# y-scope/pinot

Hardware: AMD Instinct MI355X
Metric: scanned rows/sec + achieved HBM GB/s, filtered SUM on 1B-row segment (higher is better)
Workload: dtype int64

## Files before the change

pinot_amd/csrc/pg_device.h:

```cpp
#pragma once
#include <stdint.h>

namespace pg {

constexpr int kWave = 64;
constexpr int kMaxTileSteps = 32;
constexpr int kMaxTileDocs = kWave * kMaxTileSteps;
constexpr int kMaxCols = 16;
constexpr int kMaxLeaves = 8;
constexpr int kMaxNodes = 24;
constexpr int kMaxAggCols = 4;
constexpr int kMaxGroupCols = 10;
constexpr int kMaxHashLevels = 8;
constexpr int kMaxGroupAggs = 8;
constexpr int kStackDepth = 8;
constexpr int kSetLdsWords = 2048;
constexpr int kBlockThreads = 256;
constexpr int kWideBlockThreads = 640;
constexpr int kHistBlockThreads = 1024;
constexpr unsigned long long kPartialHistAlarm = 1ull;
constexpr unsigned long long kPartialStale = 2ull;
constexpr int kGroupBlockThreads = 1024;

enum LeafKind : int32_t {
// ... 124 lines not shown
struct ScanParams {
  int32_t num_docs;
  int32_t num_tiles;
  int32_t tile_steps;
  int32_t num_cols;
  int32_t num_leaves;
  int32_t num_nodes;
  int32_t num_agg_cols;
  int32_t num_bitmap_leaves;
  int32_t stage_bytes;
  int32_t queue_off;
  int32_t queue_cap;
  int32_t wave_lds_bytes;
  int32_t speculate;
  int32_t double_buffer;
  int32_t lazy_columns;
  int32_t lazy_node;
  int32_t profile;
  int32_t bitmap_off;
  int32_t bitmap_bytes;
  int32_t num_stage;
  int32_t hist_slot;
  int32_t hist_bins;
  DevStage stage[kMaxCols];
  DevNode nodes[kMaxNodes];
  DevAggCol agg_cols[kMaxAggCols];
  const unsigned long long* bitmaps[kMaxLeaves];
  int32_t bitmap_lds_off[kMaxLeaves];
  const uint32_t* tile_list;
  const uint32_t* tile_count;
  int32_t raw64_coalesced;
  int32_t lane_skip;
  unsigned long long* filter_entries;
  unsigned long long* out_bitmap;
  BlockPartial* partials;
  uint32_t* done_counter;
  struct HostRecord* host_out;
  unsigned long long host_seq;
  int32_t fold_slots;
  int32_t fold_typed;
  int32_t sparse_lanes;
  int32_t fold_one_counter;
  uint8_t* leap_tables;
  uint32_t* leaf_out[kMaxLeaves];
  int32_t leaf_out_enabled;
  uint32_t* fsm_tables;
  int32_t fsm_states, fsm_inputs;
  int8_t fsm_input_of_leaf[kMaxLeaves];
  const struct WindowInfo* sparse_windows;
  int32_t sparse_num_windows;
  int32_t set_leaves_in_lds;
  uint8_t fsm_delta[64];
  int32_t lean_kind;
};

constexpr int kMaxDistinctKeys = 4;
struct DistinctCol {
  const uint8_t* fwd;
  uint32_t* set_bits;
  int32_t bits;
  int32_t words;
  int32_t lds_off;
  int32_t pad;
};
struct DistinctKey {
  const uint8_t* fwd;
  int32_t bits;
  uint32_t mult;
};
struct DistinctParams {
  ScanParams scan;
  int32_t num_cols;
  int32_t num_keys;
  int32_t lds_words;
  int32_t pad;
  DistinctCol cols[kMaxAggCols];
  DistinctKey keys[kMaxDistinctKeys];
};

struct CollectParams {
  DistinctParams d;
  const uint8_t* fwd[kMaxAggCols];
  int32_t vkind[kMaxAggCols];
  unsigned long long* out_images[kMaxAggCols];
  uint32_t* out_rows;
  unsigned long long* cursor;
  uint32_t* flags;
  unsigned long long capacity;
};
constexpr uint32_t kCollectOverflow = 1u;

struct HllParams {
  DistinctParams d;
  const uint8_t* fwd[kMaxAggCols];
  uint32_t* regs[kMaxAggCols];
  int32_t wide[kMaxAggCols];
  int32_t log2m[kMaxAggCols];
  int32_t lds_off[kMaxAggCols];
  int32_t lds_words;
  uint32_t num_rows;
};
enum HllDictKind : int32_t { kHllDictI32 = 0, kHllDictI64 = 1, kHllDictFloat = 2, kHllDictDouble = 3 };
struct HllFoldParams {
  const uint32_t* bits;
  uint32_t* regs;
  const int32_t* dict32;
// ... 186 lines not shown
```

pinot_amd/csrc/pg_dma_pairs.h:

```cpp
#pragma once
#include <cstddef>

namespace pg {

constexpr int kDmaMaxBits = 20;
constexpr int kDmaSlotsPerWave = 2;
constexpr int kDmaWavesPerBlock = 4;
constexpr int kDmaRecordBytes = 1024;
constexpr size_t kDmaLdsBudget = 156 * 1024;
constexpr int kDmaMinSlotBytes = 6912;
constexpr int kDmaBlocksPerCu = 2;

constexpr int dma_pieces(int bits) { return (bits + 3) / 4; }
constexpr int dma_last_lanes(int bits) { return 16 * (bits - 4 * (dma_pieces(bits) - 1)); }
constexpr int dma_instructions(int filter_bits, int value_bits) { return dma_pieces(filter_bits) + dma_pieces(value_bits); }
constexpr int dma_slot_bytes(int filter_bits, int value_bits) { return 256 * (filter_bits + value_bits); }
constexpr size_t dma_lds_bytes(int filter_bits, int value_bits, int slots, int waves) {
  return (size_t)kDmaRecordBytes + (size_t)waves * slots * dma_slot_bytes(filter_bits, value_bits);
}

constexpr bool dma_width(int bits) { return bits >= 1 && bits <= kDmaMaxBits; }
constexpr bool dma_pair_admitted(int filter_bits, int value_bits) {
  return dma_width(filter_bits) && dma_width(value_bits) && dma_slot_bytes(filter_bits, value_bits) >= kDmaMinSlotBytes &&
         kDmaLdsBudget / dma_lds_bytes(filter_bits, value_bits, kDmaSlotsPerWave, kDmaWavesPerBlock) >= (size_t)kDmaBlocksPerCu;
}
constexpr int dma_pair_index(int filter_bits, int value_bits) {
  if (!dma_pair_admitted(filter_bits, value_bits)) return -1;
  int at = 0;
  for (int f = 1; f <= kDmaMaxBits; ++f)
    for (int v = 1; v <= kDmaMaxBits; ++v) {
      if (f == filter_bits && v == value_bits) return at;
      if (dma_pair_admitted(f, v)) ++at;
    }
  return -1;
}
constexpr int dma_pair_count() {
  int n = 0;
  for (int f = 1; f <= kDmaMaxBits; ++f)
    for (int v = 1; v <= kDmaMaxBits; ++v) n += dma_pair_admitted(f, v) ? 1 : 0;
  return n;
}
constexpr int kDmaPairs = dma_pair_count();
constexpr int dma_pair_at(int index) {
  int at = 0;
  for (int f = 1; f <= kDmaMaxBits; ++f)
    for (int v = 1; v <= kDmaMaxBits; ++v)
      if (dma_pair_admitted(f, v) && at++ == index) return f * 32 + v;
  return 0;
}
static_assert(kDmaPairs == 102, "27 <= f + v <= 38, both up to 20 bits");
static_assert(dma_pair_admitted(10, 17) && dma_pair_admitted(7, 20) && dma_pair_admitted(20, 18) && !dma_pair_admitted(6, 20) && !dma_pair_admitted(19, 20), "the rule's edges");

}
```

pinot_amd/csrc/pg_engine.hip:

```cpp
#include <hip/hip_runtime.h>

#include <algorithm>
#include <chrono>
#include <array>
#include <atomic>
#include <condition_variable>
#include <functional>
#include <memory>
#include <cmath>
#include <cstdarg>
#include <cstdio>
#include <cstdlib>
#include <cstring>
#include <limits>
#include <mutex>
#include <string>
#include <thread>
#include <vector>

#include "../../include/pinot_gpu.h"
#include "pg_device.h"
#include "pg_filter_stats.h"
#include "pg_filter_fsm.h"
#include "pg_fsm_kernels.h"
#include "pg_kernels.h"
#include "pg_launch.h"
#include "pg_rank_image.h"
#include "pg_raw_set_table.h"
#include "pg_hll.h"
#include "pg_set_pass_layout.h"
#include "pg_group_plan.h"
#include "pg_dma_pairs.h"
#include "pg_chunk_decode.h"

namespace {

using namespace pg;

thread_local std::string g_error;

pg_status fail(pg_status st, const char* fmt, ...) {
  char buf[1024];
  va_list ap;
  va_start(ap, fmt);
  vsnprintf(buf, sizeof(buf), fmt, ap);
  va_end(ap);
  g_error = buf;
  return st;
}

#define HIP_TRY(expr)                                                                                  \
  do {                                                                                                 \
    hipError_t _e = (expr);                                                                            \
    if (_e != hipSuccess)                                                                              \
      return fail(_e == hipErrorOutOfMemory ? PG_ERR_OUT_OF_MEMORY : PG_ERR_DEVICE, "%s failed: %s (%s:%d)", #expr, \
                  hipGetErrorString(_e), __FILE__, __LINE__);                                          \
  } while (0)

struct Engine {
  bool initialized = false;
  std::atomic<uint64_t> epoch{0};
  int device = 0;
  int blocks_per_cu = 0;
  bool raw64_coalesced = true;
  int wide_plane = -1;
  bool partition_stats_cache = true;
  bool partition_packed = true;
  bool plane_async = true;
  bool staged_h2d = true;
  long long exact_stats_docs = 64ll << 20;
  int flags = 0;
  bool use_dma = true;
  int value_plane = -1;
  int tile_steps = 0;
  bool double_buffer = false;
  bool direct_result = true;
  int fold_finalize = -1;
  int fold_one_counter = 1;
  bool poll_result = true;
  bool distinct_lds = true;
  bool collect = false;
  bool chunk_decode_host = false;
  bool percentile_lds = true;
  bool set_lds = true;
  bool lane_skip = true;
  bool batch_blocks_per_cu_forced = false;
  int batch_blocks_per_cu = 4;
  bool scan_raw = true;
  bool scan_raw_set = true;
  int scan_simple_valid = 1;
  int scan_simple_pipe = 1;
  int scan_simple_dma = 1;
  int dma_pair = 1;
  int dma_nt = -1;
  int dma_blocks_per_cu = 0;
  bool scan_simple = true;
  bool scan_sparse = true;
  bool lean_batch = true;
  bool partition_two_level = true;
  bool fsm_perm = true;
  int index_and_waves = 0;
  bool batch_index = true;
  bool index_gather = true;
  bool fsm_fused = true;
  bool fsm_stats = true;
  bool fsm_episodes = true;
  bool plan_cache = true;
  bool group_publish = true;
  bool batch_more = true;
  bool group_one_launch = true;
  bool batch_group = true;
  bool batch_hist = true;
  bool batch_launch = true;
  bool leap2 = true;
  int sparse_lanes = 32;
  bool plane_gcd = true;
  bool scan_private = true;
  bool group_private = true;
  int group_log_replicas = 3;
  bool group_pack = true;
  bool scan_typed_private = true;
  bool scan_narrow_single = true;
  bool scan_narrow = true;
  bool group_partition = true;
  long long partition_min_docs = 1ll << 22;
  unsigned long long group_table_bytes = 64ull << 30;
  int hist = -1;
  int hist_blocks = 0;
  bool hist_guard = false;
  int hist_bits = 0;
// ... 146 lines not shown
  mutable std::mutex doc_sets_mu;
  std::vector<std::shared_ptr<DocSet>> doc_sets;
};


struct FsmSide {
  const pg::fstats::Fsm* fsm = nullptr;
  uint32_t* bitmap[pg::kFsmInputs] = {};
  bool mapped[pg::kFsmInputs] = {};
  bool kernel_wrote = false;
  uint32_t* tables = nullptr;
  uint32_t* chunks = nullptr;
  unsigned long long* entries = nullptr;
  long long num_tiles = 0, num_chunks = 0;
  bool fused = false;
  bool prepared = false;
};
constexpr size_t kAndShardBytes = (size_t)pg::kAndCardinalityShards * 128;
constexpr size_t kFsmStageBytes = 64 + (1 + (size_t)fstats::kFsmMaxEpisodeStreams) * ((size_t)pg::kFsmStates << pg::kFsmInputs);

namespace {

void destroy_ctx(ExecCtx* c) {
  if (!c) return;
  if (c->stream) (void)hipStreamSynchronize(c->stream);
  if (c->h_fsm_stage) (void)hipHostFree(c->h_fsm_stage);
  if (c->d_fsm_scratch) (void)hipFree(c->d_fsm_scratch);
  for (hipEvent_t e : c->ev_pass) if (e) (void)hipEventDestroy(e);
  if (c->d_partials) (void)hipFree(c->d_partials);
  if (c->h_record) (void)hipHostFree(c->h_record);
  if (c->d_done) (void)hipFree(c->d_done);
  for (auto* b : c->d_bitmaps) (void)hipFree(b);
  for (auto* s : c->d_sets) (void)hipFree(s);
  if (c->d_table) (void)hipFree(c->d_table);
  if (c->h_table) (void)hipHostFree(c->h_table);
  if (c->d_gather_in) (void)hipFree(c->d_gather_in);
  if (c->d_gather_out) (void)hipFree(c->d_gather_out);
  if (c->d_partition) (void)hipFree(c->d_partition);
  if (c->d_tile_list) (void)hipFree(c->d_tile_list);
  if (c->d_and_counters) (void)hipFree(c->d_and_counters);
  if (c->h_and_shards) (void)hipHostFree(c->h_and_shards);
  if (c->d_window_info) (void)hipFree(c->d_window_info);
  if (c->d_distinct) (void)hipFree(c->d_distinct);
  if (c->d_arena) (void)hipFree(c->d_arena);
  if (c->h_groups) (void)hipHostFree(c->h_groups);
  if (c->d_filter_entries) (void)hipFree(c->d_filter_entries);
  if (c->d_leap_tables) (void)hipFree(c->d_leap_tables);
  if (c->h_filter_entries) (void)hipHostFree(c->h_filter_entries);
  for (auto& e : c->ev) if (e) (void)hipEventDestroy(e);
  if (c->stream) (void)hipStreamDestroy(c->stream);
  delete c;
}

pg_status acquire_ctx(pg_segment* seg, ExecCtx** out) {
  {
    std::lock_guard<std::mutex> lk(seg->ctx_mu);
    if (!seg->free_ctx.empty()) {
      *out = seg->free_ctx.back();
      seg->free_ctx.pop_back();
      return PG_OK;
    }
  }
  ExecCtx* c = new ExecCtx();
  hipError_t e = hipStreamCreateWithFlags(&c->stream, hipStreamNonBlocking);
  if (e == hipSuccess) for (auto& ev : c->ev) { e = hipEventCreate(&ev); if (e != hipSuccess) break; }
  if (e == hipSuccess) e = hipHostMalloc((void**)&c->h_record, sizeof(HostRecord), hipHostMallocMapped);
  if (e == hipSuccess) { memset(c->h_record, 0, sizeof(HostRecord)); c->h_partial = &c->h_record->partial; }
  if (e == hipSuccess) e = hipHostGetDevicePointer((void**)&c->h_record_dev, c->h_record, 0);
  if (e == hipSuccess) e = hipMalloc((void**)&c->d_done, 10 * 128);
  if (e == hipSuccess) e = hipMemsetAsync(c->d_done, 0, 10 * 128, c->stream);
  if (e != hipSuccess) {
    destroy_ctx(c);
    return fail(PG_ERR_DEVICE, "creating execution context failed: %s", hipGetErrorString(e));
  }
  {
    std::lock_guard<std::mutex> lk(seg->ctx_mu);
    seg->all_ctx.push_back(c);
  }
  *out = c;
  return PG_OK;
}

void release_ctx(pg_segment* seg, ExecCtx* c) {
  std::lock_guard<std::mutex> lk(seg->ctx_mu);
  seg->free_ctx.push_back(c);
}

struct CtxGuard {
  pg_segment* seg;
  ExecCtx* ctx;
  ~CtxGuard() { if (ctx) release_ctx(seg, ctx); }
};

pg_status ensure_partials(ExecCtx* c, int blocks) {
  if (c->partial_capacity >= blocks + kFoldExtraRecords) return PG_OK;
  if (c->d_partials) (void)hipFree(c->d_partials);
  c->d_partials = nullptr;
  HIP_TRY(hipMalloc((void**)&c->d_partials, sizeof(BlockPartial) * (size_t)(blocks + kFoldExtraRecords)));
  c->partial_capacity = blocks + kFoldExtraRecords;
  return PG_OK;
}

pg_status ensure_bitmap(pg_segment* seg, ExecCtx* c, size_t index) {
  while (c->d_bitmaps.size() <= index) {
    unsigned long long* p = nullptr;
    size_t words = (size_t)std::max(seg->num_tiles, 1) * kMaxTileSteps;
    HIP_TRY(hipMalloc((void**)&p, words * 8));
    c->d_bitmaps.push_back(p);
  }
  return PG_OK;
}

constexpr size_t kDistinctKeepWords = (size_t)64 << 20;
pg_status ensure_distinct(pg_segment* seg, ExecCtx* c, size_t words) {
  if (c->distinct_capacity >= words) return PG_OK;
  if (c->d_distinct) { (void)hipFree(c->d_distinct); seg->device_bytes -= c->distinct_capacity * 4; }
  c->d_distinct = nullptr; c->distinct_capacity = 0;
  HIP_TRY(hipMalloc((void**)&c->d_distinct, words * 4));
  c->distinct_capacity = words;
  seg->device_bytes += words * 4;
  return PG_OK;
}
void trim_distinct(pg_segment* seg, ExecCtx* c) {
// ... 1338 lines not shown
#else
  std::this_thread::yield();
#endif
}

template <typename Done>
pg_status wait_polled(hipStream_t stream, long long docs, Done&& done) {
  long long spins = 0;
  std::chrono::steady_clock::time_point until;
  while (!done()) {
    cpu_relax();
    if ((++spins & 0x3FF) != 0) continue;
    const auto now = std::chrono::steady_clock::now();
    if (spins == 0x400) { until = now + std::chrono::nanoseconds(300'000 + docs / 1000); continue; }
    if (now >= until || hipStreamQuery(stream) != hipErrorNotReady) { HIP_TRY(hipStreamSynchronize(stream)); break; }
  }
  __atomic_thread_fence(__ATOMIC_ACQUIRE);
  return PG_OK;
}

}

extern "C" {

const char* pg_last_error(void) { return g_error.c_str(); }
const char* pg_version(void) { return "pinot_amd 0.1 (gfx950)"; }

pg_status pg_init(const pg_config* config) {
  std::lock_guard<std::mutex> lk(g_engine.mu);
  if (config && config->abi_version != PG_ABI_VERSION) return fail(PG_ERR_INVALID_ARGUMENT, "ABI version mismatch: got %d, built %d", config->abi_version, PG_ABI_VERSION);
  int count = 0;
  hipError_t e = hipGetDeviceCount(&count);
  if (e != hipSuccess || count == 0) return fail(PG_ERR_DEVICE, "no HIP device available: %s", hipGetErrorString(e));
  g_engine.physical_devices = count;
  const char* ald = getenv("PINOT_GPU_ALIAS_DEVICES");
  g_engine.logical_devices = (ald && atoi(ald) > count) ? std::min(atoi(ald), 64) : count;
  int dev = config ? config->device_id : 0;
  if (dev < 0 || dev >= g_engine.logical_devices) return fail(PG_ERR_INVALID_ARGUMENT, "device %d out of range (have %d)", dev, g_engine.logical_devices);
  g_engine.device = dev;
  g_engine.blocks_per_cu = config ? config->blocks_per_cu : 0;
  g_engine.flags = config ? config->flags : 0;
  const char* nodma = getenv("PINOT_GPU_NO_DMA");
  g_engine.use_dma = !(nodma && nodma[0] == '1');
  const char* vp = getenv("PINOT_GPU_VALUE_PLANE");
  g_engine.value_plane = vp ? atoi(vp) : -1;
  const char* db = getenv("PINOT_GPU_DOUBLE_BUFFER");
  g_engine.double_buffer = db && db[0] == '1';
  const char* drv = getenv("PINOT_GPU_DIRECT_RESULT");
  g_engine.direct_result = !(drv && drv[0] == '0');
  const char* ffz = getenv("PINOT_GPU_FOLD_FINALIZE");
  g_engine.fold_finalize = ffz ? (ffz[0] == '0' ? 0 : 1) : -1;
  const char* foc = getenv("PINOT_GPU_FOLD_ONE_COUNTER");
  g_engine.fold_one_counter = foc ? (foc[0] == '0' ? 0 : 1) : 1;
  const char* prs = getenv("PINOT_GPU_POLL_RESULT");
  g_engine.poll_result = !(prs && prs[0] == '0');
  const char* lsk = getenv("PINOT_GPU_LANE_SKIP");
  g_engine.lane_skip = !(lsk && lsk[0] == '0');
  const char* bbc = getenv("PINOT_GPU_BATCH_BLOCKS_PER_CU");
  g_engine.batch_blocks_per_cu_forced = bbc != nullptr;
  g_engine.batch_blocks_per_cu = (bbc && atoi(bbc) > 0) ? atoi(bbc) : 4;
  const char* ssp = getenv("PINOT_GPU_SCAN_SPARSE");
  g_engine.scan_sparse = !(ssp && ssp[0] == '0');
  const char* ssm = getenv("PINOT_GPU_SCAN_SIMPLE");
  g_engine.scan_simple = !(ssm && ssm[0] == '0');
  const char* ssv = getenv("PINOT_GPU_SCAN_SIMPLE_VALID");
  g_engine.scan_simple_valid = ssv ? (ssv[0] == '0' ? 0 : (ssv[0] == '2' ? 2 : 1)) : 1;
  const char* spp = getenv("PINOT_GPU_SCAN_SIMPLE_PIPE");
  g_engine.scan_simple_pipe = spp ? (spp[0] == '0' ? 0 : (spp[0] == '2' ? 2 : 1)) : 1;
  const char* sdm = getenv("PINOT_GPU_SCAN_SIMPLE_DMA");
  g_engine.scan_simple_dma = sdm ? (sdm[0] == '0' ? 0 : (sdm[0] == '2' ? 2 : 1)) : 1;
  const char* sdp = getenv("PINOT_GPU_SCAN_SIMPLE_DMA_PAIR");
  g_engine.dma_pair = sdp && sdp[0] == '0' ? 0 : 1;
  const char* sdn = getenv("PINOT_GPU_SCAN_SIMPLE_DMA_NT");
  g_engine.dma_nt = sdn ? (sdn[0] == '0' ? 0 : 1) : -1;
  const char* sdb = getenv("PINOT_GPU_SCAN_SIMPLE_DMA_BLOCKS_PER_CU");
  g_engine.dma_blocks_per_cu = sdb && atoi(sdb) > 0 ? atoi(sdb) : 0;
  const char* srw = getenv("PINOT_GPU_SCAN_RAW");
  g_engine.scan_raw = !(srw && srw[0] == '0');
  const char* srs = getenv("PINOT_GPU_SCAN_RAW_SET");
  g_engine.scan_raw_set = !(srs && srs[0] == '0');
  const char* bla = getenv("PINOT_GPU_BATCH_LAUNCH");
  g_engine.batch_launch = !(bla && bla[0] == '0');
  auto env_on = [](const char* name) { const char* v = getenv(name); return !(v && v[0] == '0'); };
  g_engine.lean_batch = env_on("PINOT_GPU_LEAN_BATCH");
  g_engine.set_lds = env_on("PINOT_GPU_SET_LDS");
  g_engine.distinct_lds = env_on("PINOT_GPU_DISTINCT_LDS");
  g_engine.percentile_lds = env_on("PINOT_GPU_PERCENTILE_LDS");
  { const char* cv = getenv("PINOT_GPU_COLLECT"); g_engine.collect = cv != nullptr && cv[0] == '1'; }
  { const char* cd = getenv("PINOT_GPU_CHUNK_DECODE"); g_engine.chunk_decode_host = cd != nullptr && strcmp(cd, "host") == 0; }
  g_engine.partition_two_level = env_on("PINOT_GPU_PARTITION_TWO_LEVEL");
  g_engine.fsm_perm = env_on("PINOT_GPU_FSM_PERM");
  g_engine.fsm_stats = env_on("PINOT_GPU_FSM_STATS");
  g_engine.fsm_fused = env_on("PINOT_GPU_FSM_FUSED");
  g_engine.fsm_episodes = env_on("PINOT_GPU_FSM_EPISODES");
  g_engine.index_gather = env_on("PINOT_GPU_INDEX_GATHER");
  g_engine.batch_index = env_on("PINOT_GPU_BATCH_INDEX");
  { const char* iaw = getenv("PINOT_GPU_INDEX_AND_WAVES"); g_engine.index_and_waves = iaw ? std::max(-64, std::min(32, atoi(iaw))) : 0; }
  g_engine.group_one_launch = env_on("PINOT_GPU_GROUP_ONE_LAUNCH");
  g_engine.plan_cache = env_on("PINOT_GPU_PLAN_CACHE");
  g_engine.group_publish = env_on("PINOT_GPU_GROUP_PUBLISH");
  const char* bmo = getenv("PINOT_GPU_BATCH_MORE");
  g_engine.batch_more = !(bmo && bmo[0] == '0');
  const char* bgr = getenv("PINOT_GPU_BATCH_GROUP");
  g_engine.batch_group = !(bgr && bgr[0] == '0');
  const char* bhi = getenv("PINOT_GPU_BATCH_HIST");
  g_engine.batch_hist = !(bhi && bhi[0] == '0');
// ... 1768 lines not shown
      const int ac = agg_slot_of[(size_t)a];
      const ColumnDev& col = seg->cols[(size_t)ag.column];
      const bool plane = lw.plane_cols[(size_t)ag.column] != 0;
      const bool raw = col.encoding == PG_FWD_RAW_FIXED_BYTE;
      if (ag.function == PG_AGG_SUM || ag.function == PG_AGG_AVG) {
        if (col.vkind == kValF64 || col.vkind == kValF32) {
          v.sum = fp.fsum[ac];
          v.sum_i64 = 0;
          v.sum_exact = 0;
        } else if (col.vkind == kValI64) {
          v.sum_i64 = fp.sum[ac];
          const bool wrapped = std::fabs(fp.fsum[ac] - (double)fp.sum[ac]) > 4.6e18;
          v.sum_exact = wrapped ? 0 : 1;
          v.sum = wrapped ? fp.fsum[ac] : (double)v.sum_i64;
        } else {
          set_integer_sum(&v, (__int128)fp.sum[ac] * (__int128)sum_scale(col, plane) + (__int128)fp.count * (__int128)sum_base(col, plane));
        }
      } else if (fp.count > 0) {
        if (raw && col.vkind != kValI32) {
          double mn = key64_to_double(col, fp.kmin64[ac]), mx = key64_to_double(col, fp.kmax64[ac]);
          if (mx != mx) mn = mx;
          if (ag.function == PG_AGG_MIN) v.min = mn;
          if (ag.function == PG_AGG_MAX) v.max = mx;
        } else {
          if (ag.function == PG_AGG_MIN) v.min = agg_value_double(col, fp.kmin[ac], plane);
          if (ag.function == PG_AGG_MAX) v.max = agg_value_double(col, fp.kmax[ac], plane);
          if (dict_ends_in_nan(col) && fp.kmax[ac] == col.cardinality - 1) {
            if (ag.function == PG_AGG_MIN) v.min = col.h_dict_f64.back();
          }
        }
      }
    }
    out->dominant_kernel = kernel_id;
    for (int c = 0; c < 4; ++c) out->profile_cycles[c] = fp.cyc[c];
    out->profile_waves = profile_waves;
    out->stats.num_docs_scanned = (int64_t)fp.count;
    finish_filter_stats(lw, seg, (int64_t)fp.entries + (count_leap2 ? host_record->leap_correction : 0), count_entries, out);
    out->stats.num_entries_scanned_post_filter = (int64_t)fp.count * (int64_t)num_projected;
    out->stats.num_total_docs = seg->num_docs;
  };
  const bool folded = g_engine.fold_finalize >= 0 ? g_engine.fold_finalize != 0 : true;
  sp.done_counter = folded ? ctx->d_done : nullptr;
  sp.host_out = g_engine.direct_result ? ctx->h_record_dev : nullptr;
  sp.host_seq = seq;
  sp.fold_slots = k.kernel == ScanKernel::Hist ? 2 : pl.num_agg_cols;
  sp.fold_typed = (k.kernel == ScanKernel::PrivateTyped || (k.kernel == ScanKernel::Agg && typed)) ? 1 : 0;
  sp.lane_skip = g_engine.lane_skip ? 1 : 0;
  sp.set_leaves_in_lds = 0;
  if (g_engine.set_lds) for (int nd = 0; nd < sp.num_nodes; ++nd) if (sp.nodes[nd].op == PG_FILTER_LEAF && sp.nodes[nd].kind == kLeafDictSet) sp.set_leaves_in_lds = 1;
  if (k.kernel == ScanKernel::Hist || pass.form != SetPass::None) sp.set_leaves_in_lds = grid.hist_set_off != 0 ? 1 + (int32_t)grid.hist_set_off : 0;
  if (pass.form != SetPass::None) { st = arm_set_pass(r, &pass, grid); if (st != PG_OK) return st; }
  sp.sparse_lanes = g_engine.sparse_lanes;
  sp.fold_one_counter = g_engine.fold_one_counter;
  if (defer_index_and) {
    auto item = index_and_item(lw);
    item->one_slot = pl.num_agg_cols <= 1;
    item->convert = convert;
    return defer_item(r, std::move(item));
  }
  BatchKind kind = BatchKind::Private;
  if (r.defer != nullptr && !r.defer->single && scan_batch_kind(k, pl.num_agg_cols, &kind) && !want_bitmap && out && sp.tile_list == nullptr && !count_entries &&
      !ctx->pre_enqueued && g_engine.direct_result && lw.side == nullptr && doc_tiles(seg) <= kBatchMaxTiles && r.stats_is_final) {
    sp.lean_kind = (int32_t)kind;
    auto item = std::make_shared<LoweredItem>();
    item->sp = sp;
    item->blocks = blocks;
    item->one_slot = pl.num_agg_cols <= 1;
    item->convert = convert;
    item->sets = lw.set_leaves;
    if (k.kernel == ScanKernel::Hist) { item->hist_lds = grid.lds; item->hist_cw = k.hist_cw; item->hist_col = r.hist_col; }
    return defer_item(r, std::move(item));
  }
  if (lw.gathered) {
    HIP_TRY(hipMemcpyAsync(ctx->h_and_shards, ctx->d_and_counters + 2, kAndShardBytes, hipMemcpyDeviceToHost, ctx->stream));
    if (timed) HIP_TRY(hipEventRecord(ctx->ev[3], ctx->stream));
    ctx->ev_last = 3;
    exec_mark(3);
    HIP_TRY(hipStreamSynchronize(ctx->stream));
    exec_mark(4);
    BlockPartial g;
    st = read_index_and_shards(ctx, pl.num_agg_cols, &g); if (st != PG_OK) return st;
    *ctx->h_partial = g;
  } else {
    const bool post_work = !g_engine.direct_result || count_leap2 || want_bitmap || sp.leaf_out_enabled || k.kernel == ScanKernel::PrivateFsm || pass.form != SetPass::None;
    if (timed) HIP_TRY(hipEventRecord(ctx->ev[1], ctx->stream));
    if (pass.form != SetPass::None) launch_set_pass(r, &pass, grid);
    else launch_scan_kernel(k, grid, pl.num_agg_cols, typed, ctx->stream, sp);
    HIP_TRY(hipGetLastError());
    if (timed) HIP_TRY(hipEventRecord(ctx->ev[2], ctx->stream));
    if (pass.form != SetPass::None) { st = enqueue_set_pass_post(r, &pass); if (st != PG_OK) return st; }
    if (!folded) {
      finalize_partials_kernel<<<dim3(1), dim3(kBlockThreads), 0, ctx->stream>>>(ctx->d_partials, blocks, g_engine.direct_result ? ctx->h_record_dev : nullptr, seq,
                                                                                  sp.fold_slots, sp.fold_typed, sp.profile);
      HIP_TRY(hipGetLastError());
    }
    if (!g_engine.direct_result) HIP_TRY(hipMemcpyAsync(ctx->h_partial, ctx->d_partials + blocks, sizeof(BlockPartial), hipMemcpyDeviceToHost, ctx->stream));
    if (count_leap2) { st = launch_leap_chain(seg, ctx, seq); if (st != PG_OK) return st; }
    if (k.kernel == ScanKernel::PrivateFsm) {
      const FsmSide& fs = *lw.side;
      fsm_chain_kernel<<<dim3((unsigned)fs.num_chunks), dim3(1024), 0, ctx->stream>>>(fs.tables, fs.num_tiles, sp.fsm_states, fs.chunks);
      HIP_TRY(hipGetLastError());
      fsm_finish_kernel<<<dim3(1), dim3(1024), (size_t)fs.num_chunks * (size_t)sp.fsm_states * 4, ctx->stream>>>(fs.chunks, (int)fs.num_chunks, sp.fsm_states, fs.entries);
      HIP_TRY(hipGetLastError());
      HIP_TRY(hipMemcpyAsync(ctx->h_filter_entries, fs.entries, 8, hipMemcpyDeviceToHost, ctx->stream));
    }
    if (want_bitmap) {
      const int64_t need = ((int64_t)seg->num_docs + 63) / 64;
      if (d_out_bitmap_request) {
        if (need) HIP_TRY(hipMemcpyAsync(d_out_bitmap_request, ctx->d_bitmaps[0], (size_t)need * 8, hipMemcpyDeviceToDevice, ctx->stream));
      } else {
        if (host_bitmap_words < need) return fail(PG_ERR_INVALID_ARGUMENT, "bitmap buffer has %lld words, need %lld", (long long)host_bitmap_words, (long long)need);
        if (need) HIP_TRY(hipMemcpyAsync(host_bitmap, ctx->d_bitmaps[0], (size_t)need * 8, hipMemcpyDeviceToHost, ctx->stream));
      }
    }
    if (timed && (post_work || !folded)) HIP_TRY(hipEventRecord(ctx->ev[3], ctx->stream));
    ctx->ev_last = (post_work || !folded) ? 3 : 2;
    exec_mark(3);
    if (g_engine.poll_result && !post_work && !timed) {
      volatile unsigned long long* flag = &ctx->h_record->seq;
      st = wait_polled(ctx->stream, (long long)seg->num_docs, [&] { return *flag == seq; }); if (st != PG_OK) return st;
      if (*flag != seq) return fail(PG_ERR_INTERNAL, "the scan kernel finished without publishing its record");
    } else {
      HIP_TRY(hipStreamSynchronize(ctx->stream));
    }
    exec_mark(4);
    if (count_leap2 && ctx->h_record->leap_seq != seq) return fail(PG_ERR_INTERNAL, "the leap-frog chain kernel did not publish its result");
    if (g_engine.direct_result && ctx->h_record->seq != seq) return fail(PG_ERR_INTERNAL, "the scan kernel's record carries sequence %llu, expected %llu", ctx->h_record->seq, seq);
  }
  const BlockPartial& fp = *ctx->h_partial;
  if (fp.flags & kPartialStale) return fail(PG_ERR_INTERNAL, "the scan kernel's fold read a record that was not written by this launch (sequence %llu)", seq);
  const bool hist_wrapped = k.kernel == ScanKernel::Hist && !k.hist_guarded && k.hist_cw < 32 && (unsigned long long)fp.sum[1] != fp.count;
  if (k.kernel == ScanKernel::Hist && (hist_wrapped || (fp.flags & kPartialHistAlarm))) {
    __atomic_store_n(&seg->cols[(size_t)r.hist_col].hist_tier, hist_wrapped ? 1 : 2, __ATOMIC_RELAXED);
    seg->plane_epoch.fetch_add(1, std::memory_order_acq_rel);
    return kHistRetry;
  }
  if (out_cardinality) *out_cardinality = (int64_t)fp.count;
  if (out) convert(fp, out);
  if (pass.form != SetPass::None) { st = harvest_set_pass(r, &pass, fp); if (st != PG_OK) return st; }
  if (out && k.kernel == ScanKernel::PrivateFsm) {
    out->stats.num_entries_scanned_in_filter = (int64_t)*ctx->h_filter_entries;
    out->filter_entries_exact = 1;
    lw.side->fused = true;
  }
  return PG_OK;
}
enum class GroupRoute { Partition, TypedDirect, Private, Staged };
struct GroupPlan {
  GroupParams gp;
  std::vector<int> cards;
  int group_slot[kMaxGroupCols] = {}, group_mult[kMaxGroupCols] = {};
  PlanGroupAgg plan_aggs[kMaxGroupAggs];
  std::vector<int> dev_agg_of;
  HashPlan hash_plan; long long product = 1;
  bool no_dict_keys = false;
  bool first_appearance = false, map_based = false, private_leaves = true;
  size_t table_words = 0, table_bytes = 0; Geometry geo;
  int pblocks = 1, pthreads = kBlockThreads; size_t plds = 0;
  PartitionPlan part; int packed_bits = 0;
  GroupRoute route = GroupRoute::Staged;
  bool count_leap2 = false, count_entries = false;
  GroupPlan() { memset(&gp, 0, sizeof(gp)); }
  bool private_sized() const { return route == GroupRoute::Partition || route == GroupRoute::Private; }
  bool route_writes_leaf_outputs() const { return route == GroupRoute::Private || route == GroupRoute::TypedDirect; }
  int kernel_id() const { return route == GroupRoute::Partition ? PG_KERNEL_GROUP_PARTITION : (route == GroupRoute::Private ? PG_KERNEL_GROUP_PRIVATE : PG_KERNEL_SCAN_GROUP); }
};
static inline void decode_mixed_radix(long long raw, const std::vector<int>& cards, int ng, int32_t* out) {
  for (int g = 0; g < ng; ++g) { out[g] = (int32_t)(raw % cards[(size_t)g]); raw /= cards[(size_t)g]; }
}
static void group_agg_value(const pg_segment* seg, const pg_aggregation& ag, bool plane, long long acc, unsigned long long group_docs, pg_agg_value* v) {
  const ColumnDev& col = seg->cols[(size_t)ag.column];
  if (ag.function == PG_AGG_SUM || ag.function == PG_AGG_AVG) {
    if (col.vkind == kValF64 || col.vkind == kValF32) { memcpy(&v->sum, &acc, 8); v->sum_i64 = 0; v->sum_exact = 0; }
    else set_integer_sum(v, (__int128)acc * (__int128)sum_scale(col, plane) + (__int128)group_docs * (__int128)sum_base(col, plane));
  }
  else if (col.encoding == PG_FWD_RAW_FIXED_BYTE && col.vkind != kValI32) {
    if (ag.function == PG_AGG_MIN) v->min = group_key64_to_double(col, acc, true); else v->max = group_key64_to_double(col, acc, false);
  }
  else if (ag.function == PG_AGG_MIN) v->min = group_dict_min_double(col, (int32_t)acc, plane);
  else v->max = agg_value_double(col, (int32_t)acc, plane);
// ... 2669 lines not shown
```

pinot_amd/csrc/pg_scan_simple_dma.h:

```cpp
#pragma once
#include "pg_dma_pairs.h"
#include "pg_scan_simple.h"

namespace pg {

typedef const __attribute__((address_space(3))) uint32_t* LdsWords;

static_assert(sizeof(BlockPartial) * (kBlockThreads / 64) + 16 <= kDmaRecordBytes, "the records and the flag fit their area");
static_assert(kDmaMaxBits == kSimpleMaxBits && kDmaWavesPerBlock == kBlockThreads / 64, "pg_dma_pairs.h speaks of this kernel's widths and workgroups");

template <int J> __device__ __forceinline__ void dma_wait() { asm volatile("s_waitcnt vmcnt(%0)" :: "n"(J) : "memory"); }

template <int N, int kAux>
__device__ __forceinline__ void dma_stage_tile(const uint8_t* f_tile, const uint8_t* v_tile, int f_bytes, int v_bytes, int nf, uint8_t* slot, int lane) {
#pragma unroll
  for (int j = 0; j < N; ++j) {
    const bool is_f = j < nf;
    const int at = (is_f ? j : j - nf) * 1024, chunk = is_f ? f_bytes : v_bytes;
    const uint8_t* src = (is_f ? f_tile : v_tile) + at + lane * 16;
    uint8_t* dst = slot + (is_f ? 0 : f_bytes) + at;
    if (at + lane * 16 < chunk)
      __builtin_amdgcn_global_load_lds((const __attribute__((address_space(1))) void*)src, (__attribute__((address_space(3))) void*)dst, 16, 0, kAux);
  }
}

template <typename P>
__device__ __forceinline__ void dma_tile(const P& p, long long tile, int lane, const uint8_t* slot, unsigned long long& count, unsigned long long& sum,
                                         uint32_t& umin, uint32_t& umax) {
  const auto& L = p.nodes[0];
  const auto& ac = p.agg_cols[0];
  const LdsWords fw = (LdsWords)(const uint32_t*)slot + lane * L.bits;
  const LdsWords vw = (LdsWords)(const uint32_t*)(slot + 256 * L.bits) + lane * ac.bits;
  uint32_t m = L.lo == 0 ? simple_range_dispatch<true>(L.bits, fw, 0u, L.span) : simple_range_dispatch<false>(L.bits, fw, (uint32_t)L.lo, L.span);
  if (L.exclusive) m = ~m;
  const long long rem = (long long)p.num_docs - (tile * 2048 + lane * 32);
  m &= rem >= 32 ? 0xFFFFFFFFu : (rem <= 0 ? 0u : ((1u << (int)rem) - 1u));
  count += (unsigned)__builtin_popcount(m);
  uint32_t psum = 0, tmin = 0xFFFFFFFFu, tmax = 0u;
  unsigned long long wsum = 0;
  simple_agg_dispatch(ac.bits, vw, m, ac.need_sum != 0, ac.need_minmax != 0, psum, wsum, tmin, tmax);
  sum += wsum + psum;
  umin = tmin < umin ? tmin : umin;
  umax = tmax > umax ? tmax : umax;
}

template <int N, int S, int kAux, typename P>
__device__ __forceinline__ void scan_simple_dma_body(const P& p, uint32_t block_index, uint32_t num_blocks, uint8_t* lds) {
  static_assert(S >= 2 && N * (S - 1) <= 63, "vmcnt counts to 63");
  BlockPartial* red = reinterpret_cast<BlockPartial*>(lds);
  uint32_t* fold_flag_ptr = reinterpret_cast<uint32_t*>(lds + sizeof(BlockPartial) * (kBlockThreads / 64));
  const int lane = threadIdx.x & 63;
  const int wave_in_block = __builtin_amdgcn_readfirstlane((int)(threadIdx.x >> 6));
  const int waves_per_block = blockDim.x >> 6;
  const long long total_waves = (long long)num_blocks * waves_per_block;
  const long long num_tiles = ((long long)p.num_docs + 2047) / 2048;
  const auto& L = p.nodes[0];
  const auto& ac = p.agg_cols[0];
  const int f_bytes = 256 * L.bits, v_bytes = 256 * ac.bits, slot_bytes = f_bytes + v_bytes, nf = (L.bits + 3) >> 2;
  uint8_t* ring = lds + kDmaRecordBytes + (size_t)wave_in_block * S * slot_bytes;

  unsigned long long count = 0, sum = 0;
  uint32_t umin = 0xFFFFFFFFu, umax = 0u;
  const long long first = (long long)block_index * waves_per_block + wave_in_block;
  const long long n = first < num_tiles ? (num_tiles - first + total_waves - 1) / total_waves : 0;
#pragma unroll
  for (int k = 0; k < S - 1; ++k)
    if (k < n) dma_stage_tile<N, kAux>(L.fwd + (first + k * total_waves) * f_bytes, ac.fwd + (first + k * total_waves) * v_bytes, f_bytes, v_bytes, nf, ring + k * slot_bytes, lane);
  long long i = 0, tile = first;
  int rd = 0, wr = S - 1;
  for (; i + (S - 1) < n; ++i, tile += total_waves) {
    asm volatile("s_waitcnt lgkmcnt(0)" ::: "memory");
    const long long ahead = tile + (S - 1) * total_waves;
    dma_stage_tile<N, kAux>(L.fwd + ahead * f_bytes, ac.fwd + ahead * v_bytes, f_bytes, v_bytes, nf, ring + wr * slot_bytes, lane);
    dma_wait<N * (S - 1)>();
    dma_tile(p, tile, lane, ring + rd * slot_bytes, count, sum, umin, umax);
    rd = rd + 1 == S ? 0 : rd + 1;
    wr = wr + 1 == S ? 0 : wr + 1;
  }
#define PG_DMA_DRAIN(R) if (S - 1 >= R && n - i == R) { dma_wait<N * (R - 1)>(); dma_tile(p, tile, lane, ring + rd * slot_bytes, count, sum, umin, umax); \
                          rd = rd + 1 == S ? 0 : rd + 1; ++i; tile += total_waves; }
  PG_DMA_DRAIN(3) PG_DMA_DRAIN(2) PG_DMA_DRAIN(1)
#undef PG_DMA_DRAIN
  static_assert(S <= 4, "PG_DMA_DRAIN covers rings of up to four slots");

  BlockPartial mine;
  partial_identity(mine);
  mine.count = (unsigned long long)wave_sum_i64((long long)count);
  mine.sum[0] = wave_sum_i64((long long)sum);
  mine.kmin[0] = wave_min_i32(umin == 0xFFFFFFFFu ? 0x7FFFFFFF : (int32_t)umin);
  mine.kmax[0] = wave_max_i32(count == 0ull ? (int32_t)0x80000000 : (int32_t)umax);
  if (lane == 0) red[wave_in_block] = mine;
  __syncthreads();
  publish_block_partial(p, red, waves_per_block, fold_flag_ptr, block_index, num_blocks);
}

template <int B, int J, int kAux>
__device__ __forceinline__ void dma_stage_piece(const uint8_t* src, uint8_t* dst, int lane) {
  constexpr int base = J >= 4 ? 4096 : 0, off = (J & 3) * 1024;
  if (J + 1 < dma_pieces(B) || dma_last_lanes(B) == 64 || lane < dma_last_lanes(B))
    __builtin_amdgcn_global_load_lds((const __attribute__((address_space(1))) void*)(src + base), (__attribute__((address_space(3))) void*)(dst + base), 16, off, kAux);
}
template <int B, int kAux>
__device__ __forceinline__ void dma_stage_column(const uint8_t* src, uint8_t* dst, int lane) {
  static_assert(dma_pieces(B) <= 5, "columns of up to 20 bits");
  dma_stage_piece<B, 0, kAux>(src, dst, lane);
  if constexpr (dma_pieces(B) > 1) dma_stage_piece<B, 1, kAux>(src, dst, lane);
  if constexpr (dma_pieces(B) > 2) dma_stage_piece<B, 2, kAux>(src, dst, lane);
  if constexpr (dma_pieces(B) > 3) dma_stage_piece<B, 3, kAux>(src, dst, lane);
  if constexpr (dma_pieces(B) > 4) dma_stage_piece<B, 4, kAux>(src, dst, lane);
}

template <int FB, int VB, bool kLoZero, bool kMinMax>
__device__ __forceinline__ void dma_pair_tile(const uint8_t* slot, int lane, uint32_t lo, uint32_t span, uint32_t flip, long long rem,
                                              unsigned long long& count, unsigned long long& sum, uint32_t& umin, uint32_t& umax) {
  const LdsWords fw = (LdsWords)(const uint32_t*)slot + lane * FB;
  const LdsWords vw = (LdsWords)(const uint32_t*)(slot + 256 * FB) + lane * VB;
  uint32_t fd[FB], vd[VB];
#pragma unroll
  for (int i = 0; i < FB; ++i) fd[i] = fw[i];
#pragma unroll
  for (int i = 0; i < VB; ++i) vd[i] = vw[i];
  uint32_t m = 0;
  range16_private<FB, 0, kLoZero>((const uint32_t*)fd, lo, span, m);
  range16_private<FB, 1, kLoZero>((const uint32_t*)fd, lo, span, m);
  m = __builtin_bitreverse32(m) ^ flip;
  m &= rem >= 32 ? 0xFFFFFFFFu : (rem <= 0 ? 0u : ((1u << (int)rem) - 1u));
  count += (unsigned)__builtin_popcount(m);
  uint32_t psum = 0, tmin = 0xFFFFFFFFu, tmax = 0u;
  unsigned long long wsum = 0;
  agg16_private<VB, 0>((const uint32_t*)vd, m, true, kMinMax, psum, wsum, tmin, tmax);
  agg16_private<VB, 1>((const uint32_t*)vd, m, true, kMinMax, psum, wsum, tmin, tmax);
  sum += wsum + psum;
  umin = tmin < umin ? tmin : umin;
  umax = tmax > umax ? tmax : umax;
}

template <int FB, int VB, int kAux, bool kLoZero, bool kMinMax, typename P>
__device__ __forceinline__ void dma_pair_tiles(const P& p, long long first, uint32_t n, long long total_waves, uint8_t* ring, int lane,
                                               unsigned long long& count, unsigned long long& sum, uint32_t& umin, uint32_t& umax) {
  constexpr int f_bytes = 256 * FB, v_bytes = 256 * VB, slot_bytes = f_bytes + v_bytes, N = dma_instructions(FB, VB);
  const auto& L = p.nodes[0];
  const uint32_t lo = (uint32_t)L.lo, span = L.span, flip = L.exclusive ? 0xFFFFFFFFu : 0u;
  const uint32_t lane_at = (uint32_t)lane * 16u;
  const uint8_t* f_next = L.fwd + first * f_bytes;
  const uint8_t* v_next = p.agg_cols[0].fwd + first * v_bytes;
  const long long f_step = total_waves * f_bytes, v_step = total_waves * v_bytes;
  long long rem = (long long)p.num_docs - (first * 2048 + lane * 32);
  const long long rem_step = total_waves * 2048;
  if (n > 0) {
    dma_stage_column<FB, kAux>(f_next + lane_at, ring, lane);
    dma_stage_column<VB, kAux>(v_next + lane_at, ring + f_bytes, lane);
  }
  int rd = 0;
  for (uint32_t i = 0; i < n; ++i, rem -= rem_step) {
    if (i + 1 < n) {
      asm volatile("s_waitcnt lgkmcnt(0)" ::: "memory");
      f_next += f_step; v_next += v_step;
      uint8_t* wr = ring + (slot_bytes - rd);
      dma_stage_column<FB, kAux>(f_next + lane_at, wr, lane);
      dma_stage_column<VB, kAux>(v_next + lane_at, wr + f_bytes, lane);
      dma_wait<N>();
    } else {
      dma_wait<0>();
    }
    dma_pair_tile<FB, VB, kLoZero, kMinMax>(ring + rd, lane, lo, span, flip, rem, count, sum, umin, umax);
    rd = slot_bytes - rd;
  }
}

template <int FB, int VB, int kAux, typename P>
__device__ __forceinline__ void scan_simple_dma_pair_body(const P& p, uint32_t block_index, uint32_t num_blocks, uint8_t* lds) {
  static_assert(kDmaSlotsPerWave == 2 && dma_instructions(FB, VB) <= 63, "two slots; vmcnt counts to 63");
  BlockPartial* red = reinterpret_cast<BlockPartial*>(lds);
  uint32_t* fold_flag_ptr = reinterpret_cast<uint32_t*>(lds + sizeof(BlockPartial) * (kBlockThreads / 64));
  const int lane = threadIdx.x & 63;
  const int wave_in_block = __builtin_amdgcn_readfirstlane((int)(threadIdx.x >> 6));
  const int waves_per_block = blockDim.x >> 6;
  const long long total_waves = (long long)num_blocks * waves_per_block;
  const long long num_tiles = ((long long)p.num_docs + 2047) / 2048;
  uint8_t* ring = lds + kDmaRecordBytes + (size_t)wave_in_block * kDmaSlotsPerWave * dma_slot_bytes(FB, VB);

  unsigned long long count = 0, sum = 0;
  uint32_t umin = 0xFFFFFFFFu, umax = 0u;
  const long long first = (long long)block_index * waves_per_block + wave_in_block;
  const uint32_t n = first < num_tiles ? (uint32_t)((num_tiles - first + total_waves - 1) / total_waves) : 0u;
  const bool lo_zero = p.nodes[0].lo == 0, need_sum = p.agg_cols[0].need_sum != 0, need_minmax = p.agg_cols[0].need_minmax != 0;
#define PG_PAIR_TILES(Z, M) dma_pair_tiles<FB, VB, kAux, Z, M>(p, first, n, total_waves, ring, lane, count, sum, umin, umax)
  if (lo_zero) { if (need_sum && !need_minmax) PG_PAIR_TILES(true, false); else PG_PAIR_TILES(true, true); }
  else { if (need_sum && !need_minmax) PG_PAIR_TILES(false, false); else PG_PAIR_TILES(false, true); }
#undef PG_PAIR_TILES
  if (!need_sum) sum = 0;
  if (!need_minmax) { umin = 0xFFFFFFFFu; umax = 0u; }

  BlockPartial mine;
  partial_identity(mine);
  mine.count = (unsigned long long)wave_sum_i64((long long)count);
  mine.sum[0] = wave_sum_i64((long long)sum);
  mine.kmin[0] = wave_min_i32(umin == 0xFFFFFFFFu ? 0x7FFFFFFF : (int32_t)umin);
  mine.kmax[0] = wave_max_i32(count == 0ull ? (int32_t)0x80000000 : (int32_t)umax);
  if (lane == 0) red[wave_in_block] = mine;
  __syncthreads();
  publish_block_partial(p, red, waves_per_block, fold_flag_ptr, block_index, num_blocks);
}


}
```

Baseline: 1915 billion.

## Fold DMA scan totals through sharded device atomics instead of per-block partial records

```diff
diff --git a/pinot_amd/csrc/pg_device.h b/pinot_amd/csrc/pg_device.h
--- a/pinot_amd/csrc/pg_device.h
+++ b/pinot_amd/csrc/pg_device.h
@@ -200,6 +200,7 @@
   int32_t set_leaves_in_lds;
   uint8_t fsm_delta[64];
   int32_t lean_kind;
+  unsigned long long* ring_totals;
 };
 
 constexpr int kMaxDistinctKeys = 4;
diff --git a/pinot_amd/csrc/pg_dma_pairs.h b/pinot_amd/csrc/pg_dma_pairs.h
--- a/pinot_amd/csrc/pg_dma_pairs.h
+++ b/pinot_amd/csrc/pg_dma_pairs.h
@@ -10,6 +10,8 @@
 constexpr size_t kDmaLdsBudget = 156 * 1024;
 constexpr int kDmaMinSlotBytes = 6912;
 constexpr int kDmaBlocksPerCu = 2;
+constexpr int kRingTotalShards = 8, kRingTotalWords = 3, kRingTotalStride = 16;
+constexpr size_t kRingTotalsBytes = (size_t)kRingTotalShards * kRingTotalStride * 8;
 
 constexpr int dma_pieces(int bits) { return (bits + 3) / 4; }
 constexpr int dma_last_lanes(int bits) { return 16 * (bits - 4 * (dma_pieces(bits) - 1)); }
diff --git a/pinot_amd/csrc/pg_engine.hip b/pinot_amd/csrc/pg_engine.hip
--- a/pinot_amd/csrc/pg_engine.hip
+++ b/pinot_amd/csrc/pg_engine.hip
@@ -76,6 +76,7 @@
   bool double_buffer = false;
   bool direct_result = true;
   int fold_finalize = -1;
+  bool ring_totals = true;
   int fold_one_counter = 1;
   bool poll_result = true;
   bool distinct_lds = true;
@@ -328,6 +329,9 @@
   delete c;
 }
 
+constexpr size_t kDoneBytes = 10 * 128;
+static unsigned long long* ring_totals_of(const ExecCtx* c) { return reinterpret_cast<unsigned long long*>(reinterpret_cast<uint8_t*>(c->d_done) + kDoneBytes); }
+
 pg_status acquire_ctx(pg_segment* seg, ExecCtx** out) {
   {
     std::lock_guard<std::mutex> lk(seg->ctx_mu);
@@ -343,8 +347,8 @@
   if (e == hipSuccess) e = hipHostMalloc((void**)&c->h_record, sizeof(HostRecord), hipHostMallocMapped);
   if (e == hipSuccess) { memset(c->h_record, 0, sizeof(HostRecord)); c->h_partial = &c->h_record->partial; }
   if (e == hipSuccess) e = hipHostGetDevicePointer((void**)&c->h_record_dev, c->h_record, 0);
-  if (e == hipSuccess) e = hipMalloc((void**)&c->d_done, 10 * 128);
-  if (e == hipSuccess) e = hipMemsetAsync(c->d_done, 0, 10 * 128, c->stream);
+  if (e == hipSuccess) e = hipMalloc((void**)&c->d_done, kDoneBytes + kRingTotalsBytes);
+  if (e == hipSuccess) e = hipMemsetAsync(c->d_done, 0, kDoneBytes + kRingTotalsBytes, c->stream);
   if (e != hipSuccess) {
     destroy_ctx(c);
     return fail(PG_ERR_DEVICE, "creating execution context failed: %s", hipGetErrorString(e));
@@ -1789,6 +1793,8 @@
   g_engine.fold_finalize = ffz ? (ffz[0] == '0' ? 0 : 1) : -1;
   const char* foc = getenv("PINOT_GPU_FOLD_ONE_COUNTER");
   g_engine.fold_one_counter = foc ? (foc[0] == '0' ? 0 : 1) : 1;
+  const char* rgt = getenv("PINOT_GPU_RING_TOTALS");
+  g_engine.ring_totals = !(rgt && rgt[0] == '0');
   const char* prs = getenv("PINOT_GPU_POLL_RESULT");
   g_engine.poll_result = !(prs && prs[0] == '0');
   const char* lsk = getenv("PINOT_GPU_LANE_SKIP");
@@ -3663,6 +3669,7 @@
   if (pass.form != SetPass::None) { st = arm_set_pass(r, &pass, grid); if (st != PG_OK) return st; }
   sp.sparse_lanes = g_engine.sparse_lanes;
   sp.fold_one_counter = g_engine.fold_one_counter;
+  sp.ring_totals = nullptr;
   if (defer_index_and) {
     auto item = index_and_item(lw);
     item->one_slot = pl.num_agg_cols <= 1;
@@ -3694,6 +3701,10 @@
     *ctx->h_partial = g;
   } else {
     const bool post_work = !g_engine.direct_result || count_leap2 || want_bitmap || sp.leaf_out_enabled || k.kernel == ScanKernel::PrivateFsm || pass.form != SetPass::None;
+    const bool ring_totals = g_engine.ring_totals && k.kernel == ScanKernel::Simple && k.dma && folded && g_engine.direct_result && !post_work && sp.profile == 0 &&
+                             pl.num_agg_cols == 1 && sp.agg_cols[0].need_minmax == 0;
+    if (ring_totals) sp.ring_totals = ring_totals_of(ctx);
+    auto rearm_ring_totals = [&] { if (ring_totals) (void)hipMemsetAsync(ctx->d_done, 0, kDoneBytes + kRingTotalsBytes, ctx->stream); };
     if (timed) HIP_TRY(hipEventRecord(ctx->ev[1], ctx->stream));
     if (pass.form != SetPass::None) launch_set_pass(r, &pass, grid);
     else launch_scan_kernel(k, grid, pl.num_agg_cols, typed, ctx->stream, sp);
@@ -3729,14 +3740,17 @@
     exec_mark(3);
     if (g_engine.poll_result && !post_work && !timed) {
       volatile unsigned long long* flag = &ctx->h_record->seq;
-      st = wait_polled(ctx->stream, (long long)seg->num_docs, [&] { return *flag == seq; }); if (st != PG_OK) return st;
-      if (*flag != seq) return fail(PG_ERR_INTERNAL, "the scan kernel finished without publishing its record");
+      st = wait_polled(ctx->stream, (long long)seg->num_docs, [&] { return *flag == seq; }); if (st != PG_OK) { rearm_ring_totals(); return st; }
+      if (*flag != seq) { rearm_ring_totals(); return fail(PG_ERR_INTERNAL, "the scan kernel finished without publishing its record"); }
     } else {
-      HIP_TRY(hipStreamSynchronize(ctx->stream));
+      const hipError_t waited = hipStreamSynchronize(ctx->stream);
+      if (waited != hipSuccess) rearm_ring_totals();
+      HIP_TRY(waited);
     }
     exec_mark(4);
     if (count_leap2 && ctx->h_record->leap_seq != seq) return fail(PG_ERR_INTERNAL, "the leap-frog chain kernel did not publish its result");
-    if (g_engine.direct_result && ctx->h_record->seq != seq) return fail(PG_ERR_INTERNAL, "the scan kernel's record carries sequence %llu, expected %llu", ctx->h_record->seq, seq);
+    if (g_engine.direct_result && ctx->h_record->seq != seq) { rearm_ring_totals(); return fail(PG_ERR_INTERNAL, "the scan kernel's record carries sequence %llu, expected %llu", ctx->h_record->seq, seq); }
+    if (ctx->h_partial->flags & kPartialStale) rearm_ring_totals();
   }
   const BlockPartial& fp = *ctx->h_partial;
   if (fp.flags & kPartialStale) return fail(PG_ERR_INTERNAL, "the scan kernel's fold read a record that was not written by this launch (sequence %llu)", seq);
diff --git a/pinot_amd/csrc/pg_scan_simple_dma.h b/pinot_amd/csrc/pg_scan_simple_dma.h
--- a/pinot_amd/csrc/pg_scan_simple_dma.h
+++ b/pinot_amd/csrc/pg_scan_simple_dma.h
@@ -44,6 +44,76 @@
   umax = tmax > umax ? tmax : umax;
 }
 
+static_assert(kRingTotalShards == kFoldShards && kRingTotalWords == 3, "pg_dma_pairs.h sizes the area: a shard per arrival shard; count, sum, stamp");
+struct RingStamps { unsigned long long arrived = 0, fold_begin = 0, seq_stored = 0; };
+template <bool kStamps, typename P>
+__device__ __forceinline__ void publish_ring_totals(const P& p, BlockPartial* red, int waves_per_block, uint32_t* flag, uint32_t block_index, uint32_t num_blocks,
+                                                    RingStamps& stamps) {
+  const bool one_counter = p.fold_one_counter != 0 && num_blocks <= (uint32_t)kFoldOneCounterMax;
+  const uint32_t shard = block_index & (kFoldShards - 1);
+  const uint32_t arrive_at = one_counter ? 0u : shard;
+  const uint32_t in_shard = one_counter ? num_blocks : (num_blocks + (kFoldShards - 1) - shard) / kFoldShards;
+  const uint32_t shards = num_blocks < (uint32_t)kFoldShards ? num_blocks : (uint32_t)kFoldShards;
+  if (threadIdx.x == 0) {
+    unsigned long long count = red[0].count, sum = (unsigned long long)red[0].sum[0];
+    for (int w = 1; w < waves_per_block; ++w) { count += red[w].count; sum += (unsigned long long)red[w].sum[0]; }
+    unsigned long long* mine = p.ring_totals + shard * kRingTotalStride;
+    (void)__hip_atomic_fetch_add(mine + 0, count, __ATOMIC_RELAXED, __HIP_MEMORY_SCOPE_AGENT);
+    (void)__hip_atomic_fetch_add(mine + 1, sum, __ATOMIC_RELAXED, __HIP_MEMORY_SCOPE_AGENT);
+    (void)__hip_atomic_fetch_add(mine + 2, p.host_seq, __ATOMIC_RELAXED, __HIP_MEMORY_SCOPE_AGENT);
+    asm volatile("s_waitcnt vmcnt(0)" ::: "memory");
+    uint32_t go = __hip_atomic_fetch_add(p.done_counter + arrive_at * kFoldStride, 1u, __ATOMIC_RELAXED, __HIP_MEMORY_SCOPE_AGENT) + 1u == in_shard ? 1u : 0u;
+    if (go != 0u && !one_counter)
+      go = __hip_atomic_fetch_add(p.done_counter + kFoldShards * kFoldStride, 1u, __ATOMIC_RELAXED, __HIP_MEMORY_SCOPE_AGENT) + 1u == shards ? 1u : 0u;
+    if constexpr (kStamps) stamps.arrived = wall_clock64();
+    *flag = go;
+  }
+  __syncthreads();
+  if (*flag == 0u || threadIdx.x >= 64) return;
+  if (threadIdx.x == 0) {
+    if constexpr (kStamps) stamps.fold_begin = wall_clock64();
+    unsigned long long t[kRingTotalWords] = {0ull, 0ull, 0ull};
+#pragma unroll
+    for (int s = 0; s < kFoldShards; ++s)
+#pragma unroll
+      for (int w = 0; w < kRingTotalWords; ++w) t[w] += __hip_atomic_load(p.ring_totals + s * kRingTotalStride + w, __ATOMIC_RELAXED, __HIP_MEMORY_SCOPE_AGENT);
+#pragma unroll
+    for (int s = 0; s < kFoldShards; ++s)
+#pragma unroll
+      for (int w = 0; w < kRingTotalWords; ++w) __hip_atomic_store(p.ring_totals + s * kRingTotalStride + w, 0ull, __ATOMIC_RELAXED, __HIP_MEMORY_SCOPE_AGENT);
+    for (int c = 0; c <= kFoldShards; ++c) __hip_atomic_store(p.done_counter + c * kFoldStride, 0u, __ATOMIC_RELAXED, __HIP_MEMORY_SCOPE_AGENT);
+    BlockPartial acc;
+    partial_identity(acc);
+    acc.count = t[0];
+    acc.sum[0] = (long long)t[1];
+    acc.kmax[0] = t[0] == 0ull ? (int32_t)0x80000000 : 0;
+    acc.flags = t[2] != (unsigned long long)num_blocks * p.host_seq ? kPartialStale : 0ull;
+    acc.stamp = p.host_seq;
+    red[0] = acc;
+  }
+  store_host_record_by_wave0(p.host_out, &red[0], p.host_seq);
+  if constexpr (kStamps) if (threadIdx.x == 0) stamps.seq_stored = wall_clock64();
+}
+
+template <bool kStamps, typename P>
+__device__ __forceinline__ void publish_ring(const P& p, BlockPartial* red, int waves_per_block, uint32_t* flag, uint32_t block_index, uint32_t num_blocks,
+                                             unsigned long long* stamps_out, const unsigned long long (&wave_stamps)[3]) {
+  RingStamps rs;
+  const bool totals = p.ring_totals != nullptr && num_blocks > 1u;
+  if (totals) publish_ring_totals<kStamps>(p, red, waves_per_block, flag, block_index, num_blocks, rs);
+  else publish_block_partial(p, red, waves_per_block, flag, block_index, num_blocks);
+  if constexpr (kStamps) {
+    const unsigned long long left = wall_clock64();
+    if ((threadIdx.x & 63) == 0) {
+      unsigned long long* w = stamps_out + ((size_t)block_index * waves_per_block + (threadIdx.x >> 6)) * 6;
+      w[0] = wave_stamps[0]; w[1] = wave_stamps[1]; w[2] = wave_stamps[2];
+      w[3] = totals && threadIdx.x == 0 ? rs.arrived : left;
+      w[4] = threadIdx.x == 0 ? (totals ? rs.fold_begin : (*flag != 0u ? 1ull : 0ull)) : 0ull;
+      w[5] = threadIdx.x == 0 ? (totals ? rs.seq_stored : (*flag != 0u ? left : 0ull)) : 0ull;
+    }
+  }
+}
+
 template <int N, int S, int kAux, typename P>
 __device__ __forceinline__ void scan_simple_dma_body(const P& p, uint32_t block_index, uint32_t num_blocks, uint8_t* lds) {
   static_assert(S >= 2 && N * (S - 1) <= 63, "vmcnt counts to 63");
@@ -91,7 +161,8 @@
   mine.kmax[0] = wave_max_i32(count == 0ull ? (int32_t)0x80000000 : (int32_t)umax);
   if (lane == 0) red[wave_in_block] = mine;
   __syncthreads();
-  publish_block_partial(p, red, waves_per_block, fold_flag_ptr, block_index, num_blocks);
+  const unsigned long long no_stamps[3] = {0ull, 0ull, 0ull};
+  publish_ring<false>(p, red, waves_per_block, fold_flag_ptr, block_index, num_blocks, nullptr, no_stamps);
 }
 
 template <int B, int J, int kAux>
@@ -135,9 +206,9 @@
   umax = tmax > umax ? tmax : umax;
 }
 
-template <int FB, int VB, int kAux, bool kLoZero, bool kMinMax, typename P>
+template <int FB, int VB, int kAux, bool kLoZero, bool kMinMax, bool kStamps = false, typename P>
 __device__ __forceinline__ void dma_pair_tiles(const P& p, long long first, uint32_t n, long long total_waves, uint8_t* ring, int lane,
-                                               unsigned long long& count, unsigned long long& sum, uint32_t& umin, uint32_t& umax) {
+                                               unsigned long long& count, unsigned long long& sum, uint32_t& umin, uint32_t& umax, unsigned long long& landed) {
   constexpr int f_bytes = 256 * FB, v_bytes = 256 * VB, slot_bytes = f_bytes + v_bytes, N = dma_instructions(FB, VB);
   const auto& L = p.nodes[0];
   const uint32_t lo = (uint32_t)L.lo, span = L.span, flip = L.exclusive ? 0xFFFFFFFFu : 0u;
@@ -163,13 +234,16 @@
     } else {
       dma_wait<0>();
     }
+    if constexpr (kStamps) if (i == 0) landed = wall_clock64();
     dma_pair_tile<FB, VB, kLoZero, kMinMax>(ring + rd, lane, lo, span, flip, rem, count, sum, umin, umax);
     rd = slot_bytes - rd;
   }
 }
 
-template <int FB, int VB, int kAux, typename P>
-__device__ __forceinline__ void scan_simple_dma_pair_body(const P& p, uint32_t block_index, uint32_t num_blocks, uint8_t* lds) {
+template <int FB, int VB, int kAux, bool kStamps = false, typename P>
+__device__ __forceinline__ void scan_simple_dma_pair_body(const P& p, uint32_t block_index, uint32_t num_blocks, uint8_t* lds, unsigned long long* stamps_out = nullptr) {
+  unsigned long long wave_stamps[3] = {0ull, 0ull, 0ull};
+  if constexpr (kStamps) wave_stamps[0] = wall_clock64();
   static_assert(kDmaSlotsPerWave == 2 && dma_instructions(FB, VB) <= 63, "two slots; vmcnt counts to 63");
   BlockPartial* red = reinterpret_cast<BlockPartial*>(lds);
   uint32_t* fold_flag_ptr = reinterpret_cast<uint32_t*>(lds + sizeof(BlockPartial) * (kBlockThreads / 64));
@@ -185,12 +259,13 @@
   const long long first = (long long)block_index * waves_per_block + wave_in_block;
   const uint32_t n = first < num_tiles ? (uint32_t)((num_tiles - first + total_waves - 1) / total_waves) : 0u;
   const bool lo_zero = p.nodes[0].lo == 0, need_sum = p.agg_cols[0].need_sum != 0, need_minmax = p.agg_cols[0].need_minmax != 0;
-#define PG_PAIR_TILES(Z, M) dma_pair_tiles<FB, VB, kAux, Z, M>(p, first, n, total_waves, ring, lane, count, sum, umin, umax)
+#define PG_PAIR_TILES(Z, M) dma_pair_tiles<FB, VB, kAux, Z, M, kStamps>(p, first, n, total_waves, ring, lane, count, sum, umin, umax, wave_stamps[1])
   if (lo_zero) { if (need_sum && !need_minmax) PG_PAIR_TILES(true, false); else PG_PAIR_TILES(true, true); }
   else { if (need_sum && !need_minmax) PG_PAIR_TILES(false, false); else PG_PAIR_TILES(false, true); }
 #undef PG_PAIR_TILES
   if (!need_sum) sum = 0;
   if (!need_minmax) { umin = 0xFFFFFFFFu; umax = 0u; }
+  if constexpr (kStamps) { asm volatile("" :: "v"(count), "v"(sum)); wave_stamps[2] = wall_clock64(); }
 
   BlockPartial mine;
   partial_identity(mine);
@@ -200,8 +275,8 @@
   mine.kmax[0] = wave_max_i32(count == 0ull ? (int32_t)0x80000000 : (int32_t)umax);
   if (lane == 0) red[wave_in_block] = mine;
   __syncthreads();
-  publish_block_partial(p, red, waves_per_block, fold_flag_ptr, block_index, num_blocks);
-}
-
-
-}
+  publish_ring<kStamps>(p, red, waves_per_block, fold_flag_ptr, block_index, num_blocks, stamps_out, wave_stamps);
+}
+
+
+}
```

New measurement: 1936 billion (median of 5 runs). 1.01x the previous value.
